# Vanlightly/vsr-tlaplus

Measured on NVIDIA B200. Metric: unique states explored/sec (VSR.tla, shipped VSR.cfg constants), higher is better.
Workload: dtype u32

## Files before the change

### vsr-tlaplus_b200/csrc/vsr_gpu.cuh

```cuda
#ifndef VSR_GPU_CUH
#define VSR_GPU_CUH

#include <cuda_runtime.h>
#include <stdint.h>

#include "vsr_actions.h"

namespace vsr {

struct DevCounters {
    unsigned long long out_count;
    unsigned long long generated;
    unsigned long long ties;
    unsigned long long collisions;
    unsigned long long probes;
    unsigned long long viol_id;
    unsigned long long dead_id;
    unsigned long long tie_count;
    int error;
    int overflow;
    int viol_which;
    int _pad;
    unsigned long long work_next;
    unsigned long long drain_next;
    unsigned int send_count[8];
};

struct TieRec {
    uint64_t fp;
    uint64_t parent;
    uint32_t auxkey, cand, check, _pad;
};

struct RecHdr {
    uint64_t fp;
    uint64_t tm;
};
constexpr int MAX_WORLD = 8;


struct ExpandParams {
    const uint32_t* in;
    unsigned long long n_in;
    unsigned long long in_base;
    const uint32_t* in_hi;
    unsigned long long in_split;
    uint32_t* out;
    uint32_t* out_hi;
    unsigned long long out_split;
    unsigned long long out_cap;
    unsigned long long out_base;
    uint64_t* table;
    unsigned long long table_cap;
    uint64_t* trace;
    unsigned long long trace_cap;
    DevCounters* ctr;
    uint8_t* ties;
    unsigned long long tie_cap;
    const uint64_t* fp_tab;
    RunCfg run;
    int level;
    int check_deadlock;
    int rank, world, owner_shift;
    uint8_t* push[MAX_WORLD];
    unsigned long long push_cap;
    int push_direct;
    const uint8_t* drain[MAX_WORLD];
    unsigned int drain_n[MAX_WORLD];
    unsigned long long drain_total;
};

struct InsertParams {
    const uint8_t* recs;
    unsigned long long n;
    ExpandParams e;
};


__device__ __forceinline__ void cas128(uint64_t* p, uint64_t s0, uint64_t s1, uint64_t& o0, uint64_t& o1) {
    asm volatile(
        "{\n\t.reg .b128 cmp, swp, old;\n\tmov.b128 cmp, {%2, %3};\n\tmov.b128 swp, {%4, %5};\n\t"
        "atom.global.relaxed.gpu.cas.b128 old, [%6], cmp, swp;\n\tmov.b128 {%0, %1}, old;\n\t}"
        : "=l"(o0), "=l"(o1)
        : "l"(0ull), "l"(0ull), "l"(s0), "l"(s1), "l"(p)
        : "memory");
}
__device__ __forceinline__ void ld128_cg(const uint64_t* p, uint64_t& a, uint64_t& b) {
    asm volatile("ld.global.cg.v2.u64 {%0, %1}, [%2];" : "=l"(a), "=l"(b) : "l"(p) : "memory");
}
__device__ __forceinline__ uint64_t mix64(uint64_t x) {
    x ^= x >> 30; x *= 0xbf58476d1ce4e5b9ULL;
    x ^= x >> 27; x *= 0x94d049bb133111ebULL;
    x ^= x >> 31;
    return x;
}
template <class L, bool USE_VIEW, class W> VSR_HD uint32_t check_hash_t(const W& w) {
    constexpr int full = L::VIEW_BITS >> 5, rem = L::VIEW_BITS & 31;
    constexpr int nw = USE_VIEW ? (full + (rem ? 1 : 0)) : L::NW;
    uint32_t h = 0x9747b28cu;
VSR_UNROLL
    for (int i = 0; i < nw; i++) {
        uint32_t k = rdw(w, i);
        if (USE_VIEW && i == full) k &= (1u << rem) - 1u;
        h ^= k;
        h = ((h << 13) | (h >> 19)) * 5u + 0xe6546b64u;
    }
    h ^= h >> 16; h *= 0x85ebca6bu; h ^= h >> 13; h *= 0xc2b2ae35u; h ^= h >> 16;
    return h;
}
template <class L, class W> VSR_HD uint32_t check_hash(const W& w, bool use_view) {
    return use_view ? check_hash_t<L, true>(w) : check_hash_t<L, false>(w);
}

enum { INS_NEW = 0, INS_DUP = 1, INS_TIE = 2, INS_FULL = 3 };

constexpr unsigned long long GID_MASK = (1ull << 44) - 1ull, ROOT_GID = GID_MASK;
__host__ __device__ __forceinline__ uint64_t make_gid(int rank, unsigned long long local_id) { return ((uint64_t)rank << 40) | local_id; }
__host__ __device__ __forceinline__ uint64_t make_trec(uint64_t parent_gid, uint32_t cand) { return (parent_gid << 12) | (cand & 0xFFFu); }

__device__ __forceinline__ uint64_t make_meta(int level, uint32_t auxkey, uint32_t check) {
    return ((uint64_t)(uint32_t)level << 56) | ((uint64_t)(auxkey & 0xFFFFFFu) << 32) | check;
}

#ifndef VSR_BUCKET
#define VSR_BUCKET 2
#endif
struct Probe { uint64_t e[2 * VSR_BUCKET]; };
__device__ __forceinline__ void ld256_cg(const uint64_t* p, uint64_t& a, uint64_t& b, uint64_t& c, uint64_t& d) {
    asm volatile("ld.global.cg.v4.u64 {%0, %1, %2, %3}, [%4];" : "=l"(a), "=l"(b), "=l"(c), "=l"(d) : "l"(p) : "memory");
}
__device__ __forceinline__ unsigned long long table_home(unsigned long long cap, uint64_t fp) {
    return __umul64hi(fp * 0x9E3779B97F4A7C15ULL, cap / VSR_BUCKET) * VSR_BUCKET;
}
__device__ __forceinline__ void probe_load(const uint64_t* table, unsigned long long h, Probe& p) {
#if VSR_BUCKET == 1
    ld128_cg(table + 2 * h, p.e[0], p.e[1]);
#elif VSR_BUCKET == 2
    ld256_cg(table + 2 * h, p.e[0], p.e[1], p.e[2], p.e[3]);
#elif VSR_BUCKET == 4
    ld256_cg(table + 2 * h, p.e[0], p.e[1], p.e[2], p.e[3]);
    ld256_cg(table + 2 * h + 4, p.e[4], p.e[5], p.e[6], p.e[7]);
#else
#error "VSR_BUCKET must be 1, 2 or 4"
#endif
}
__device__ __forceinline__ int table_insert_from(uint64_t* table, unsigned long long cap, unsigned long long h, Probe p, uint64_t fp, uint64_t meta,
                                                 unsigned& probes, unsigned& collisions) {
    for (unsigned tries = 0;; tries++) {
        if (tries > (1u << 16)) return INS_FULL;
        probes++;
VSR_UNROLL
        for (int j = 0; j < VSR_BUCKET; j++) {
            uint64_t e0 = p.e[2 * j], e1 = p.e[2 * j + 1];
            if (e0 == 0) {
                cas128(table + 2 * (h + j), fp, meta, e0, e1);
                if (e0 == 0 && e1 == 0) return INS_NEW;
            }
            for (int again = 0; e1 == 0 && again < 64; again++) ld128_cg(table + 2 * (h + j), e0, e1);
            if (e0 == fp) {
                if ((uint32_t)e1 == (uint32_t)meta) {
                    const bool same_level = (e1 >> 56) == (meta >> 56);
                    const bool same_aux = ((e1 >> 32) & 0xFFFFFF) == ((meta >> 32) & 0xFFFFFF);
                    return (same_level && !same_aux) ? INS_TIE : INS_DUP;
                }
                collisions++;
            }
        }
        h += VSR_BUCKET;
        if (h >= cap) h = 0;
        probe_load(table, h, p);
    }
}
#if defined(VSR_EXP_CASFIRST) && VSR_BUCKET == 2
__device__ __forceinline__ int table_insert_casfirst(uint64_t* table, unsigned long long cap, unsigned long long h, uint64_t fp, uint64_t meta,
                                                     unsigned& probes, unsigned& collisions) {
    Probe p;
    cas128(table + 2 * h, fp, meta, p.e[0], p.e[1]);
    if (p.e[0] == 0 && p.e[1] == 0) { probes++; return INS_NEW; }
    if (p.e[0] == fp && (uint32_t)p.e[1] == (uint32_t)meta) {
        probes++;
        const bool same_level = (p.e[1] >> 56) == (meta >> 56);
        const bool same_aux = ((p.e[1] >> 32) & 0xFFFFFF) == ((meta >> 32) & 0xFFFFFF);
        return (same_level && !same_aux) ? INS_TIE : INS_DUP;
    }
    ld128_cg(table + 2 * (h + 1), p.e[2], p.e[3]);
    return table_insert_from(table, cap, h, p, fp, meta, probes, collisions);
}
#endif
__device__ __forceinline__ int table_insert(uint64_t* table, unsigned long long cap, uint64_t fp, uint64_t meta,
                                            unsigned& probes, unsigned& collisions) {
    const unsigned long long h = table_home(cap, fp);
    Probe p;
    probe_load(table, h, p);
    return table_insert_from(table, cap, h, p, fp, meta, probes, collisions);
}

__device__ __forceinline__ void bulk_store(void* gdst, const void* ssrc, uint32_t bytes) {
    asm volatile("fence.proxy.async.shared::cta;" ::: "memory");
    const uint32_t s = (uint32_t)__cvta_generic_to_shared(ssrc);
    asm volatile("cp.async.bulk.global.shared::cta.bulk_group [%0], [%1], %2;" ::"l"(gdst), "r"(s), "r"(bytes) : "memory");
    asm volatile("cp.async.bulk.commit_group;" ::: "memory");
    asm volatile("cp.async.bulk.wait_group.read 0;" ::: "memory");
}

template <int NW> __device__ __forceinline__ uint32_t* out_state(const ExpandParams& P, unsigned long long i) {
    return i < P.out_split ? P.out + i * NW : P.out_hi + (i - P.out_split) * NW;
}


constexpr int SCAP = 64;
#ifdef VSR_QPS
constexpr int QPS = VSR_QPS;
#else
constexpr int QPS = 10;
#endif

template <class L> struct WarpStage {
    alignas(16) uint32_t stage[SCAP * L::NW + 32];
    unsigned long long tstage[SCAP];
    int sn;
};
template <class L, int WARPS> struct BlockSmemT {
    static constexpr int NS = WARPS * 32;
    static constexpr int NG = 13;
    uint64_t fp_tab[8 * 256];
    uint32_t par[NS * (L::NW + 1)];
    static constexpr int QCAP = QPS * NS;
    uint16_t pool[QCAP];
    int qcount[NG];
    int take;
    unsigned long long round_first;
    WarpStage<L> w[WARPS];
};
template <class L> struct ExpandCfg {
    static constexpr size_t SMEM_ONE = 227 * 1024 - 512, SMEM_TWO = 113 * 1024;
    static constexpr int max_grp() { int m = 0; for (int g = 0; g < Ops<L>::NGRP; g++) m = Ops<L>::grp_size(g) > m ? Ops<L>::grp_size(g) : m; return m; }
    template <int W> static constexpr int pick_one() {
        if constexpr (W < 18) return 0;
        else if constexpr (sizeof(BlockSmemT<L, W>) <= SMEM_ONE) return W;
        else return pick_one<W - 2>();
    }
    static constexpr int W2 = sizeof(BlockSmemT<L, 16>) <= SMEM_TWO ? 16 : (sizeof(BlockSmemT<L, 12>) <= SMEM_TWO ? 12 : 8);
    static constexpr int W1 = max_grp() < 64 ? pick_one<32>() : 0;
#ifdef VSR_FORCE_WARPS
    static constexpr int WARPS = VSR_FORCE_WARPS;
#else
    static constexpr int WARPS = W1 >= 2 * W2 - 4 ? W1 : W2;
#endif
    static constexpr int BLOCKS = WARPS > 16 ? 1 : 2;
    typedef BlockSmemT<L, WARPS> Smem;
};

template <class L, bool MULTI> struct Expander {
    typedef Ops<L> O_;
    typedef typename ExpandCfg<L>::Smem Smem;
    static constexpr int WARPS = ExpandCfg<L>::WARPS, NS = Smem::NS;
    const ExpandParams& P;
    Smem& B;
    WarpStage<L>& S;
    const int lane, warp, tid;
    const uint32_t* mine = nullptr;
    bool have = false;

    __device__ Expander(const ExpandParams& p, Smem& b) : P(p), B(b), S(b.w[threadIdx.x >> 5]), lane(threadIdx.x & 31), warp(threadIdx.x >> 5), tid(threadIdx.x) {}

    static __device__ __noinline__ void flush(const ExpandParams& P, WarpStage<L>& S, int lane, int n) {
        const int sn = S.sn;
        unsigned long long base = 0;
        if (lane == 0) base = atomicAdd(&P.ctr->out_count, (unsigned long long)n);
        base = __shfl_sync(0xffffffffu, base, 0);
        if (lane < n) {
            const unsigned long long t = S.tstage[lane];
            if (t >> 63) {
                atomicMin(&P.ctr->viol_id, P.out_base + base + lane);
                S.tstage[lane] = t & ~(1ull << 63);
            }
        }
        __syncwarp();
        if (base + n > P.out_cap) {
            if (lane == 0) atomicExch(&P.ctr->overflow, 1);
        } else {
            if (lane == 0) {
                if (base + n <= P.out_split) bulk_store(P.out + base * L::NW, S.stage, (uint32_t)(n * L::BYTES));
                else if (base >= P.out_split) bulk_store(P.out_hi + (base - P.out_split) * L::NW, S.stage, (uint32_t)(n * L::BYTES));
                else {
                    const int n1 = (int)(P.out_split - base);
                    bulk_store(P.out + base * L::NW, S.stage, (uint32_t)(n1 * L::BYTES));
                    bulk_store(P.out_hi, S.stage + n1 * L::NW, (uint32_t)((n - n1) * L::BYTES));
                }
            }
            if (P.trace && lane < n && P.out_base + base + lane < P.trace_cap) P.trace[P.out_base + base + lane] = S.tstage[lane];
        }
        __syncwarp();
        const int rest = sn - n;
        for (int i0 = 0; i0 < rest * L::NW; i0 += 32) {
            const int i = i0 + lane;
            uint32_t v = 0;
            if (i < rest * L::NW) v = S.stage[n * L::NW + i];
            __syncwarp();
            if (i < rest * L::NW) S.stage[i] = v;
        }
        unsigned long long t = 0;
        if (lane < rest) t = S.tstage[n + lane];
        __syncwarp();
        if (lane < rest) S.tstage[lane] = t;
        if (lane == 0) S.sn = rest;
        __syncwarp();
    }

    typedef uint32_t* Row;
    static constexpr int gcd32(int a) { int g = 32; while (a % g) g >>= 1; return g; }
    static constexpr int SKEW_P = 32 / gcd32(L::NW);
    static __device__ __forceinline__ Row scratch(WarpStage<L>& S, int lane) { return &S.stage[(32 + lane) * L::NW + lane / SKEW_P]; }

    static __device__ __forceinline__ void push_records(const ExpandParams& P, WarpStage<L>& S, int lane, const RegRow<L::NW>& v, int send_to, uint64_t fp,
                                                        uint64_t tm) {
        const unsigned senders = __ballot_sync(0xffffffffu, send_to >= 0);
        if (!senders) return;
        constexpr int RB = L::BYTES + (int)sizeof(RecHdr), RW = RB / 4;
        constexpr int CAPREC = (32 * L::BYTES) / RB;
        static_assert(CAPREC >= 16, "two passes must cover a batch");
        int off = 0, cnt = 0, rnk = 0;
        unsigned mymask = 0;
        for (int d = 0; d < P.world; d++) {
            const unsigned m = __ballot_sync(0xffffffffu, send_to == d);
            if (send_to > d) off += __popc(m);
            if (send_to == d) { mymask = m; cnt = __popc(m); rnk = __popc(m & ((1u << lane) - 1u)); }
        }
        unsigned base = 0;
        if (send_to >= 0 && rnk == 0) base = atomicAdd(&P.ctr->send_count[send_to], (unsigned)cnt);
        base = __shfl_sync(0xffffffffu, base, mymask ? __ffs(mymask) - 1 : 0);
        const bool fits = send_to >= 0 && (unsigned long long)base + (unsigned)cnt <= P.push_cap;
        if (send_to >= 0 && !fits && rnk == 0) atomicExch(&P.ctr->overflow, 3);
        if (P.push_direct) {
            if (fits) {
                uint4* d = reinterpret_cast<uint4*>(P.push[send_to] + (size_t)(base + (unsigned)rnk) * RB);
                VSR_UNROLL
                for (int q = 0; q < L::NW / 4; q++) d[q] = make_uint4(v.w[4 * q], v.w[4 * q + 1], v.w[4 * q + 2], v.w[4 * q + 3]);
                d[L::NW / 4] = make_uint4((uint32_t)fp, (uint32_t)(fp >> 32), (uint32_t)tm, (uint32_t)(tm >> 32));
            }
            return;
        }
        const int pos = off + rnk, total = __popc(senders);
        uint32_t* sbuf = &S.stage[32 * L::NW];
        for (int lo = 0; lo < total; lo += CAPREC) {
            const int hi = lo + CAPREC < total ? lo + CAPREC : total;
            if (send_to >= 0 && pos >= lo && pos < hi) {
                uint32_t* r = sbuf + (pos - lo) * RW;
                VSR_UNROLL
                for (int j = 0; j < L::NW; j++) r[j] = v.w[j];
                r[L::NW] = (uint32_t)fp; r[L::NW + 1] = (uint32_t)(fp >> 32);
                r[L::NW + 2] = (uint32_t)tm; r[L::NW + 3] = (uint32_t)(tm >> 32);
            }
            __syncwarp();
            if (fits) {
                const int st = off > lo ? off : lo, en = off + cnt < hi ? off + cnt : hi;
                if (pos == st && st < en)
                    bulk_store(P.push[send_to] + (size_t)(base + (unsigned)(st - off)) * RB, sbuf + (st - lo) * RW, (uint32_t)((en - st) * RB));
            }
            __syncwarp();
        }
    }

    static __device__ __forceinline__ unsigned long long commit(const ExpandParams& P, WarpStage<L>& S, int lane, const RegRow<L::NW>& v, bool live, uint64_t fp,
                                                                uint32_t chk, uint32_t auxkey, unsigned long long home, const Probe& first, unsigned long long trec,
                                                                unsigned mult, bool check_inv = true) {
        unsigned gen = 0, probes = 0, coll = 0;
        int sn = S.sn;
        bool isnew = false;
        int bad = 0;
        if (live) {
            const uint64_t meta = make_meta(P.level, auxkey, chk);
            gen = mult;
#if defined(VSR_EXP_CASFIRST) && VSR_BUCKET == 2
            (void)first;
            const int r = table_insert_casfirst(P.table, P.table_cap, home, fp, meta, probes, coll);
#else
            const int r = table_insert_from(P.table, P.table_cap, home, first, fp, meta, probes, coll);
#endif
            isnew = r == INS_NEW;
            if (r == INS_FULL) atomicExch(&P.ctr->overflow, 4);
            if (isnew && check_inv) bad = O_::invariant(P.run, v);
            if (coll) atomicAdd(&P.ctr->collisions, (unsigned long long)coll);
            if (r == INS_TIE) {
                atomicAdd(&P.ctr->ties, 1ull);
                const unsigned long long t = atomicAdd(&P.ctr->tie_count, 1ull);
                if (t < P.tie_cap) {
                    TieRec rec;
                    rec.fp = fp; rec.parent = trec >> 12; rec.auxkey = auxkey; rec.cand = (uint32_t)(trec & 0xFFFu); rec.check = chk; rec._pad = 0;
                    uint8_t* dst = P.ties + t * (sizeof(TieRec) + L::BYTES);
                    *(TieRec*)dst = rec;
                    VSR_UNROLL
                    for (int j = 0; j < L::NW; j++) ((uint32_t*)(dst + sizeof(TieRec)))[j] = v.w[j];
                } else atomicExch(&P.ctr->overflow, 2);
            }
        }
        const unsigned newmask = __ballot_sync(0xffffffffu, isnew);
        __syncwarp();
        if (isnew) {
            const int slot = sn + __popc(newmask & ((1u << lane) - 1u));
            VSR_UNROLL
            for (int j = 0; j < L::NW; j++) S.stage[slot * L::NW + j] = v.w[j];
            if (bad) {
                trec |= 1ull << 63;
                atomicOr(&P.ctr->viol_which, bad);
            }
            S.tstage[slot] = trec;
        }
        sn += __popc(newmask);
        __syncwarp();
        if (lane == 0) S.sn = sn;
        __syncwarp();
        while (sn >= 32) {
            flush(P, S, lane, 32);
            sn -= 32;
        }
        return (unsigned long long)gen | ((unsigned long long)probes << 32);
    }

    static __device__ __noinline__ unsigned long long emit(const ExpandParams& P, Smem& B, WarpStage<L>& S, int lane, const Row n, int mult,
                                                           int cand, int si, bool act, bool check_inv) {
        int send_to = -1;
        uint64_t fp = 0;
        uint32_t chk = 0, auxkey = 0;
        unsigned long long home = 0, trec = 0;
        Probe first = {};
        bool live = false;
        RegRow<L::NW> v;
        if (act && mult > 0) {
            VSR_UNROLL
            for (int j = 0; j < L::NW; j++) v.w[j] = rdw(n, j);
        }
        if (act) {
            if (mult < 0) {
                atomicCAS(&P.ctr->error, 0, mult);
            } else if (mult > 0) {
                fp = fp64_view8<L>(B.fp_tab, v, P.run.use_view != 0);
                if (fp == 0) fp = 1;
                const int owner = MULTI ? owner_of(fp, P.owner_shift) : P.rank;
                trec = make_trec(make_gid(P.rank, P.in_base + B.round_first + si), (uint32_t)cand);
                if (owner == P.rank) {
                    live = true;
                    home = table_home(P.table_cap, fp);
#if !(defined(VSR_EXP_CASFIRST) && VSR_BUCKET == 2)
                    probe_load(P.table, home, first);
#endif
                    chk = check_hash<L>(v, P.run.use_view != 0);
                    auxkey = O_::aux_key(v);
                } else {
                    send_to = owner;
                }
            }
        }
        if (MULTI) {
            __syncwarp();
            push_records(P, S, lane, v, send_to, fp, trec | ((uint64_t)(unsigned)mult << 56));
        }
        return commit(P, S, lane, v, live, fp, chk, auxkey, home, first, trec, (unsigned)mult, check_inv);
    }

    struct DrainPre {
        uint64_t fp, tm;
        unsigned long long home;
        Probe first;
        const uint4* rec;
        bool have;
    };
    unsigned long long dchunk = ~0ull;
    __device__ __forceinline__ unsigned long long drain_chunks() const { return (P.drain_total + 31) / 32; }
    __device__ __forceinline__ unsigned long long drain_claim() {
        unsigned long long c = 0;
        if (lane == 0) c = atomicAdd(&P.ctr->drain_next, 1ull);
        return c;
    }
    __device__ __forceinline__ DrainPre drain_begin(unsigned long long chunk) {
        constexpr int RB = L::BYTES + (int)sizeof(RecHdr);
        DrainPre d;
        unsigned long long i = chunk * 32 + lane;
        d.have = chunk < drain_chunks() && i < P.drain_total;
        d.fp = d.tm = 0;
        d.home = 0;
        d.first = Probe{};
        d.rec = nullptr;
        if (d.have) {
            int s = 0;
            while (s < P.world - 1 && i >= P.drain_n[s]) { i -= P.drain_n[s]; s++; }
            d.rec = reinterpret_cast<const uint4*>(P.drain[s] + i * RB);
            const uint4 h = __ldcs(d.rec + L::NW / 4);
            d.fp = ((uint64_t)h.y << 32) | h.x;
            d.tm = ((uint64_t)h.w << 32) | h.z;
            d.home = table_home(P.table_cap, d.fp);
#if !(defined(VSR_EXP_CASFIRST) && VSR_BUCKET == 2)
            probe_load(P.table, d.home, d.first);
#endif
        }
        return d;
    }
    __device__ __forceinline__ void drain_end(const DrainPre& d) {
        RegRow<L::NW> v;
        uint32_t chk = 0, auxkey = 0;
        if (d.have) {
            VSR_UNROLL
            for (int q = 0; q < L::NW / 4; q++) {
                const uint4 x = __ldcs(d.rec + q);
                v.w[4 * q] = x.x; v.w[4 * q + 1] = x.y; v.w[4 * q + 2] = x.z; v.w[4 * q + 3] = x.w;
            }
            chk = check_hash<L>(v, P.run.use_view != 0);
            auxkey = O_::aux_key(v);
        }
        tally(commit(P, S, lane, v, d.have, d.fp, chk, auxkey, d.home, d.first, d.tm & ((1ull << 56) - 1ull), (unsigned)((d.tm >> 56) & 0xFu)));
    }
    __device__ void drain() {
        const unsigned long long nchunks = drain_chunks();
        if (dchunk == ~0ull) dchunk = __shfl_sync(0xffffffffu, drain_claim(), 0);
        while (dchunk < nchunks) {
            const unsigned long long nx = drain_claim();
            const DrainPre d = drain_begin(dchunk);
            drain_end(d);
            dchunk = __shfl_sync(0xffffffffu, nx, 0);
        }
    }

    static constexpr int NG = O_::NGRP;
    static __host__ __device__ constexpr int moff(int g) { int o = 0; for (int h = 0; h < g; h++) o += O_::grp_words(h); return o; }
    static constexpr int MW = moff(NG);
    static constexpr int PW = (NG + 1) / 2;
    static __host__ __device__ constexpr int max_grp() { int m = 0; for (int g = 0; g < NG; g++) m = O_::grp_size(g) > m ? O_::grp_size(g) : m; return m; }
    static constexpr int TBITS = NS <= 512 ? 9 : 10;
    static_assert(NS <= (1 << TBITS) && max_grp() < (1 << (16 - TBITS)), "pool item does not fit 16 bits");
    static_assert(max_grp() * NS < 65536, "16-bit packed counters");

    template <int G> __device__ __forceinline__ void guards(const RegRow<L::NW>& st, uint32_t* m, uint32_t* pc) {
        O_::template enabled_group<G>(P.run, st, m + moff(G));
        uint32_t c = 0;
        VSR_UNROLL
        for (int k = 0; k < O_::grp_words(G); k++) c += (uint32_t)__popc(m[moff(G) + k]);
        pc[G >> 1] += c << (16 * (G & 1));
        if constexpr (G + 1 < NG) guards<G + 1>(st, m, pc);
    }
    template <int G, bool FAST> __device__ __forceinline__ void push(uint32_t* m, const uint32_t* ex, const uint32_t* wb, int st) {
        int pos = st + (int)((wb[G >> 1] >> (16 * (G & 1))) & 0xFFFFu) + (int)((ex[G >> 1] >> (16 * (G & 1))) & 0xFFFFu);
        VSR_UNROLL
        for (int k = 0; k < O_::grp_words(G); k++) {
            uint32_t mm = m[moff(G) + k], left = 0;
            while (mm) {
                const int bit = __ffs(mm) - 1;
                mm &= mm - 1;
                if (FAST || pos < Smem::QCAP) B.pool[pos] = (uint16_t)(tid | ((k * 32 + bit) << TBITS));
                else left |= 1u << bit;
                pos++;
            }
            if (!FAST) m[moff(G) + k] = left;
        }
        if constexpr (G + 1 < NG) {
            const int nst = FAST ? st + B.qcount[G] : (st + B.qcount[G] < Smem::QCAP ? st + B.qcount[G] : Smem::QCAP);
            push<G + 1, FAST>(m, ex, wb, nst);
        }
    }
    template <int G> __device__ __forceinline__ void leftovers(uint32_t* m) {
        VSR_UNROLL
        for (int k = 0; k < O_::grp_words(G); k++) {
            while (__any_sync(0xffffffffu, m[moff(G) + k] != 0)) {
                const bool inl = m[moff(G) + k] != 0;
                int cand = 0;
                if (inl) {
                    const int bit = __ffs(m[moff(G) + k]) - 1;
                    m[moff(G) + k] &= m[moff(G) + k] - 1;
                    cand = O_::grp_begin(G) + k * 32 + bit;
                }
                tally(apply<G>(P, B, S, lane, mine, cand, tid, inl));
            }
        }
        if constexpr (G + 1 < NG) leftovers<G + 1>(m);
    }
    __device__ __forceinline__ void scan_all() {
        uint32_t m[MW], pc[PW];
        VSR_UNROLL
        for (int i = 0; i < MW; i++) m[i] = 0;
        VSR_UNROLL
        for (int i = 0; i < PW; i++) pc[i] = 0;
        if (have) {
            RegRow<L::NW> st;
            VSR_UNROLL
            for (int i = 0; i < L::NW; i++) st.w[i] = mine[i];
            guards<0>(st, m, pc);
        }
        uint32_t ex[PW], wb[PW];
        VSR_UNROLL
        for (int i = 0; i < PW; i++) ex[i] = pc[i];
        VSR_UNROLL
        for (int o = 1; o < 32; o <<= 1) {
            VSR_UNROLL
            for (int i = 0; i < PW; i++) {
                const uint32_t t = __shfl_up_sync(0xffffffffu, ex[i], o);
                if (lane >= o) ex[i] += t;
            }
        }
        uint32_t mytot = 0, anyc = 0;
        VSR_UNROLL
        for (int g = 0; g < NG; g++) {
            const uint32_t t = (__shfl_sync(0xffffffffu, ex[g >> 1], 31) >> (16 * (g & 1))) & 0xFFFFu;
            if (lane == g) mytot = t;
        }
        VSR_UNROLL
        for (int i = 0; i < PW; i++) { anyc |= pc[i]; ex[i] -= pc[i]; }
        uint32_t mybase = 0;
        if (lane < NG && mytot) mybase = (uint32_t)atomicAdd(&B.qcount[lane], (int)mytot);
        VSR_UNROLL
        for (int i = 0; i < PW; i++) wb[i] = 0;
        VSR_UNROLL
        for (int g = 0; g < NG; g++) wb[g >> 1] |= (__shfl_sync(0xffffffffu, mybase, g) & 0xFFFFu) << (16 * (g & 1));
        if (P.check_deadlock && have && !anyc) atomicMin(&P.ctr->dead_id, P.in_base + B.round_first + tid);
        __syncthreads();
#ifndef VSR_EXP_NO_PUSHFAST
        int all = 0;
        VSR_UNROLL
        for (int g = 0; g < NG; g++) all += B.qcount[g];
        if (all <= Smem::QCAP) {
            push<0, true>(m, ex, wb, 0);
            return;
        }
#endif
        push<0, false>(m, ex, wb, 0);
        uint32_t rest = 0;
        VSR_UNROLL
        for (int i = 0; i < MW; i++) rest |= m[i];
        if (__any_sync(0xffffffffu, rest != 0)) leftovers<0>(m);
    }
    template <int G> static __device__ __noinline__ unsigned long long apply(const ExpandParams& P, Smem& B, WarpStage<L>& S, int lane,
                                                                             const uint32_t* parent, int cand, int si, bool act) {
        const Row n = scratch(S, lane);
        int mult = 0;
        if (act) mult = O_::template step_grp<true, G>(P.run, parent, cand, n);
#ifdef VSR_EXP_INVSKIP
        return emit(P, B, S, lane, n, mult, cand, si, act, O_::may_falsify(G));
#else
        return emit(P, B, S, lane, n, mult, cand, si, act, true);
#endif
    }
    template <int G> static __device__ __forceinline__ unsigned long long batch(const ExpandParams& P, Smem& B, WarpStage<L>& S, int lane, int b,
                                                                                int k) {
        const bool act = lane < k;
        int cand = 0, si = 0;
        if (act) {
            const unsigned item = B.pool[b + lane];
            si = item & ((1 << TBITS) - 1);
            cand = O_::grp_begin(G) + (int)(item >> TBITS);
        }
        return apply<G>(P, B, S, lane, &B.par[si * (L::NW + 1)], cand, si, act);
    }
    unsigned long long acc_gen = 0, acc_probes = 0;
    __device__ __forceinline__ void tally(unsigned long long r) {
        acc_gen += (unsigned)r;
        acc_probes += r >> 32;
    }

    __device__ void run_round(unsigned long long first, int count) {
        const uint32_t* src = P.in + first * L::NW;
        if (first + count <= P.in_split) {
            for (int i = tid; i < count * L::NW; i += NS) B.par[(i / L::NW) * (L::NW + 1) + (i % L::NW)] = __ldg(src + i);
        } else {
            for (int i = tid; i < count * L::NW; i += NS) {
                const unsigned long long st = first + i / L::NW;
                const uint32_t* row = st < P.in_split ? P.in + st * L::NW : P.in_hi + (st - P.in_split) * L::NW;
                B.par[(i / L::NW) * (L::NW + 1) + (i % L::NW)] = __ldg(row + i % L::NW);
            }
        }
        if (tid < Smem::NG) B.qcount[tid] = 0;
        if (tid == 0) { B.round_first = first; B.take = 0; }
        __syncthreads();
        have = tid < count;
        mine = &B.par[(have ? tid : 0) * (L::NW + 1)];
        scan_all();
        __syncthreads();
        const int q = lane < Smem::NG ? B.qcount[lane] : 0;
        int inc = q;
        VSR_UNROLL
        for (int o = 1; o < 32; o <<= 1) {
            const int t = __shfl_up_sync(0xffffffffu, inc, o);
            if (lane >= o) inc += t;
        }
        const int seg_st = inc - q < Smem::QCAP ? inc - q : Smem::QCAP, seg_en = inc < Smem::QCAP ? inc : Smem::QCAP;
        const int nb = (seg_en - seg_st + 31) >> 5;
        int binc = nb;
        VSR_UNROLL
        for (int o = 1; o < 32; o <<= 1) {
            const int t = __shfl_up_sync(0xffffffffu, binc, o);
            if (lane >= o) binc += t;
        }
        const int total = __shfl_sync(0xffffffffu, binc, 31);
        for (;;) {
            int t = 0;
            if (lane == 0) t = atomicAdd(&B.take, 1);
            t = __shfl_sync(0xffffffffu, t, 0);
            if (t >= total) break;
            const int g = __popc(__ballot_sync(0xffffffffu, lane < Smem::NG && binc <= t));
            const int st = __shfl_sync(0xffffffffu, seg_st, g), en = __shfl_sync(0xffffffffu, seg_en, g);
            const int b = st + (t - __shfl_sync(0xffffffffu, binc - nb, g)) * 32;
            const int k = en - b < 32 ? en - b : 32;
            unsigned long long r;
            switch (g) {
            case 0: r = batch<0>(P, B, S, lane, b, k); break;   case 1: r = batch<1>(P, B, S, lane, b, k); break;
            case 2: r = batch<2>(P, B, S, lane, b, k); break;   case 3: r = batch<3>(P, B, S, lane, b, k); break;
            case 4: r = batch<4>(P, B, S, lane, b, k); break;   case 5: r = batch<5>(P, B, S, lane, b, k); break;
            case 6: r = batch<6>(P, B, S, lane, b, k); break;   case 7: r = batch<7>(P, B, S, lane, b, k); break;
            case 8: r = batch<8>(P, B, S, lane, b, k); break;   case 9: r = batch<9>(P, B, S, lane, b, k); break;
            case 10: r = batch<10>(P, B, S, lane, b, k); break; case 11: r = batch<11>(P, B, S, lane, b, k); break;
            default: r = batch<12>(P, B, S, lane, b, k); break;
            }
            tally(r);
        }
    }

    __device__ void finish() {
        while (S.sn > 0) flush(P, S, lane, S.sn < 32 ? S.sn : 32);
        for (int o = 16; o; o >>= 1) {
            acc_gen += __shfl_xor_sync(0xffffffffu, acc_gen, o);
            acc_probes += __shfl_xor_sync(0xffffffffu, acc_probes, o);
        }
        if (lane == 0) {
            atomicAdd(&P.ctr->generated, acc_gen);
            atomicAdd(&P.ctr->probes, acc_probes);
        }
    }
};

template <class L, bool MULTI> __global__ void __launch_bounds__(ExpandCfg<L>::WARPS * 32, ExpandCfg<L>::BLOCKS) expand_kernel(const __grid_constant__ ExpandParams P) {
    extern __shared__ __align__(128) unsigned char smem_raw[];
    typedef typename ExpandCfg<L>::Smem Smem;
    Smem& B = *reinterpret_cast<Smem*>(smem_raw);
    for (int i = threadIdx.x; i < 8 * 256; i += blockDim.x) B.fp_tab[i] = P.fp_tab[i];
    __shared__ unsigned long long next_round;
    Expander<L, MULTI> X(P, B);
    if ((threadIdx.x & 31) == 0) {
        WarpStage<L>& S = B.w[threadIdx.x >> 5];
        S.sn = 0;
    }
    const unsigned long long nrounds = (P.n_in + Smem::NS - 1) / Smem::NS;
    if (threadIdx.x == 0) next_round = atomicAdd(&P.ctr->work_next, 1ull);
    for (;;) {
        __syncthreads();
        const unsigned long long c = next_round;
        __syncthreads();
        if (c >= nrounds) break;
        if (threadIdx.x == 0) {
            next_round = atomicAdd(&P.ctr->work_next, 1ull);
            const unsigned long long nx = next_round;
            if (nx < nrounds && (nx + 1) * Smem::NS <= P.in_split) {
                const unsigned long long nfirst = nx * Smem::NS;
                const unsigned long long ncount = (P.n_in - nfirst) < (unsigned long long)Smem::NS ? (P.n_in - nfirst) : Smem::NS;
                asm volatile("cp.async.bulk.prefetch.L2.global [%0], %1;" ::"l"(P.in + nfirst * L::NW), "r"((uint32_t)(ncount * L::BYTES)) : "memory");
            }
        }
        const unsigned long long first = c * Smem::NS;
        const int count = (int)((P.n_in - first) < (unsigned long long)Smem::NS ? (P.n_in - first) : Smem::NS);
        X.run_round(first, count);
    }
    if (MULTI && P.drain_total) X.drain();
    X.finish();
}


template <class L> __global__ void __launch_bounds__(256) insert_kernel(const InsertParams Q) {
    const ExpandParams& P = Q.e;
    const unsigned long long i = (unsigned long long)blockIdx.x * blockDim.x + threadIdx.x;
    const int lane = threadIdx.x & 31;
    const bool have = i < Q.n;
    bool isnew = false;
    const uint8_t* rec = Q.recs + (have ? i : 0) * (L::BYTES + sizeof(RecHdr));
    const uint32_t* n = (const uint32_t*)rec;
    const RecHdr* h = (const RecHdr*)(rec + L::BYTES);
    unsigned probes = 0, coll = 0, nties = 0;
    unsigned long long gen = 0;
    uint64_t parent = 0;
    uint32_t cand = 0;
    if (have) {
        const uint64_t meta = make_meta(P.level, Ops<L>::aux_key(n), check_hash<L>(n, P.run.use_view != 0));
        const int r = table_insert(P.table, P.table_cap, h->fp, meta, probes, coll);
        isnew = r == INS_NEW;
        if (r == INS_FULL) atomicExch(&P.ctr->overflow, 4);
        gen = (h->tm >> 56) & 0xFu;
        parent = (h->tm >> 12) & ((1ull << 44) - 1ull);
        cand = (uint32_t)(h->tm & 0xFFFu);
        if (r == INS_TIE) {
            nties = 1;
            const unsigned long long t = atomicAdd(&P.ctr->tie_count, 1ull);
            if (t < P.tie_cap) {
                TieRec tr;
                tr.fp = h->fp; tr.parent = parent; tr.auxkey = (uint32_t)((meta >> 32) & 0xFFFFFF); tr.cand = cand;
                tr.check = (uint32_t)meta; tr._pad = 0;
                uint8_t* dst = P.ties + t * (sizeof(TieRec) + L::BYTES);
                *(TieRec*)dst = tr;
                for (int j = 0; j < L::NW; j++) ((uint32_t*)(dst + sizeof(TieRec)))[j] = n[j];
            } else atomicExch(&P.ctr->overflow, 2);
        }
    }
    for (int o = 16; o; o >>= 1) {
        gen += __shfl_xor_sync(0xffffffffu, gen, o);
        probes += __shfl_xor_sync(0xffffffffu, probes, o);
        coll += __shfl_xor_sync(0xffffffffu, coll, o);
        nties += __shfl_xor_sync(0xffffffffu, nties, o);
    }
    if (lane == 0) {
        if (gen) atomicAdd(&P.ctr->generated, gen);
        if (probes) atomicAdd(&P.ctr->probes, (unsigned long long)probes);
        if (coll) atomicAdd(&P.ctr->collisions, (unsigned long long)coll);
        if (nties) atomicAdd(&P.ctr->ties, (unsigned long long)nties);
    }
    const unsigned newmask = __ballot_sync(0xffffffffu, isnew);
    if (newmask) {
        unsigned long long base = 0;
        const int leader = __ffs(newmask) - 1;
        if (lane == leader) base = atomicAdd(&P.ctr->out_count, (unsigned long long)__popc(newmask));
        base = __shfl_sync(0xffffffffu, base, leader);
        if (isnew) {
            const unsigned long long pos = base + __popc(newmask & ((1u << lane) - 1u));
            if (pos < P.out_cap) {
                uint32_t* dst = out_state<L::NW>(P, pos);
                for (int j = 0; j < L::NW; j++) dst[j] = n[j];
                if (P.trace && P.out_base + pos < P.trace_cap) P.trace[P.out_base + pos] = make_trec(parent, cand);
                const int bad = Ops<L>::invariant(P.run, n);
                if (bad) {
                    atomicMin(&P.ctr->viol_id, P.out_base + pos);
                    atomicOr(&P.ctr->viol_which, bad);
                }
            } else atomicExch(&P.ctr->overflow, 1);
        }
    }
}

template <class L> __global__ void patch_ties_kernel(const ExpandParams P, const uint8_t* ties, unsigned long long ntie, unsigned long long n_out) {
    const unsigned long long i = (unsigned long long)blockIdx.x * blockDim.x + threadIdx.x;
    if (i >= n_out) return;
    uint32_t w[L::NW];
    uint32_t* st = out_state<L::NW>(P, i);
    for (int j = 0; j < L::NW; j++) w[j] = st[j];
    uint64_t fp = fp64_view8<L>(P.fp_tab, w, P.run.use_view != 0);
    if (fp == 0) fp = 1;
    const uint32_t chk = check_hash<L>(w, P.run.use_view != 0);
    const size_t stride = sizeof(TieRec) + L::BYTES;
    unsigned long long lo = 0, hi = ntie;
    while (lo < hi) {
        const unsigned long long mid = (lo + hi) / 2;
        if (((const TieRec*)(ties + mid * stride))->fp < fp) lo = mid + 1; else hi = mid;
    }
    for (; lo < ntie; lo++) {
        const TieRec* t = (const TieRec*)(ties + lo * stride);
        if (t->fp != fp) break;
        if (t->check != chk) continue;
        if (t->auxkey < Ops<L>::aux_key(w)) {
            const uint32_t* tw = (const uint32_t*)((const uint8_t*)t + sizeof(TieRec));
            for (int j = 0; j < L::NW; j++) { w[j] = tw[j]; st[j] = tw[j]; }
            if (P.trace && P.out_base + i < P.trace_cap) P.trace[P.out_base + i] = make_trec(t->parent, t->cand);
        }
    }
    const int bad = Ops<L>::invariant(P.run, w);
    if (bad) {
        atomicMin(&P.ctr->viol_id, P.out_base + i);
        atomicOr(&P.ctr->viol_which, bad);
    }
}

static __global__ void lookup_kernel(const uint64_t* table, unsigned long long cap, uint64_t fp, uint32_t check, unsigned long long* meta_out) {
    unsigned long long h = table_home(cap, fp);
    for (unsigned long long i = 0; i < cap; i++) {
        const uint64_t e0 = table[2 * h], e1 = table[2 * h + 1];
        if (e0 == 0) { *meta_out = 0; return; }
        if (e0 == fp && (uint32_t)e1 == check) { *meta_out = e1; return; }
        if (++h >= cap) h = 0;
    }
    *meta_out = 0;
}

struct SimParams {
    unsigned long long num_walks, seed;
    int depth;
    RunCfg run;
    unsigned long long* first_bad;
    unsigned long long* steps;
    unsigned long long* dead_ends;
    unsigned long long* probe_out;
    unsigned long long probe_walks;
    const uint64_t* fp_tab;
};
template <class L> __global__ void simulate_kernel(const SimParams Q) {
    unsigned long long steps = 0, dead = 0;
    for (unsigned long long wk = (unsigned long long)blockIdx.x * blockDim.x + threadIdx.x; wk < Q.num_walks; wk += (unsigned long long)gridDim.x * blockDim.x) {
        uint64_t rng = Q.seed ^ (wk * 0xD1B54A32D192ED03ULL);
        uint32_t a[L::NW], b[L::NW];
        Ops<L>::init((uint32_t*)a);
        unsigned long long mysteps = 0;
        for (int d = 2; d <= Q.depth; d++) {
            const int cand = Ops<L>::random_enabled(Q.run, (const uint32_t*)a, rng);
            if (cand < 0) { dead++; break; }
            if (Ops<L>::template step<true>(Q.run, (const uint32_t*)a, cand, (uint32_t*)b) <= 0) break;
            for (int j = 0; j < L::NW; j++) a[j] = b[j];
            steps++;
            mysteps++;
            if (Ops<L>::invariant(Q.run, (const uint32_t*)a)) {
                atomicMin(Q.first_bad, (wk << 16) | (unsigned long long)d);
                break;
            }
        }
        if (wk < Q.probe_walks) {
            Q.probe_out[2 * wk] = fp64_view<L>(Q.fp_tab, (const uint32_t*)a, false);
            Q.probe_out[2 * wk + 1] = mysteps;
        }
    }
    for (int o = 16; o; o >>= 1) {
        steps += __shfl_xor_sync(0xffffffffu, steps, o);
        dead += __shfl_xor_sync(0xffffffffu, dead, o);
    }
    if ((threadIdx.x & 31) == 0) {
        atomicAdd(Q.steps, steps);
        atomicAdd(Q.dead_ends, dead);
    }
}

static __global__ void probe_bench_kernel(uint64_t* table, unsigned long long cap, unsigned long long n, unsigned long long distinct,
                                   unsigned long long seed, unsigned long long* new_count, unsigned long long* probe_count) {
    unsigned long long mine_new = 0;
    unsigned probes = 0, coll = 0;
    for (unsigned long long i = (unsigned long long)blockIdx.x * blockDim.x + threadIdx.x; i < n; i += (unsigned long long)gridDim.x * blockDim.x) {
        unsigned long long z = seed + (i % distinct) * 0x9E3779B97F4A7C15ULL;
        z = (z ^ (z >> 30)) * 0xBF58476D1CE4E5B9ULL;
        z = (z ^ (z >> 27)) * 0x94D049BB133111EBULL;
        z ^= z >> 31;
        if (z == 0) z = 1;
        mine_new += table_insert(table, cap, z, make_meta(1, 0, (uint32_t)(z >> 32) | 1u), probes, coll) == INS_NEW;
    }
    for (int o = 16; o; o >>= 1) {
        mine_new += __shfl_xor_sync(0xffffffffu, mine_new, o);
        probes += __shfl_xor_sync(0xffffffffu, probes, o);
    }
    if ((threadIdx.x & 31) == 0) {
        atomicAdd(new_count, mine_new);
        atomicAdd(probe_count, (unsigned long long)probes);
    }
}

}
#endif
```

Baseline: 3.864 billion.

## Software-pipeline successor emission and write new states directly to global output

Each warp now double-buffers successor rows in shared memory and defers the hash-table insert of one batch until the next batch's successors have been generated, so the table probe load overlaps with the next step computation. The per-warp staging buffer with bulk-copy flushes is removed. New states get their output slot from an atomic right away and are stored straight to global memory with vector stores, and the invariant check moves after the insert. This adds pending-state bookkeeping and an extra settle call at the end of each round, and it trades coalesced bulk copies for scattered per-lane stores.

```diff
diff --git a/vsr-tlaplus_b200/csrc/vsr_gpu.cuh b/vsr-tlaplus_b200/csrc/vsr_gpu.cuh
--- a/vsr-tlaplus_b200/csrc/vsr_gpu.cuh
+++ b/vsr-tlaplus_b200/csrc/vsr_gpu.cuh
@@ -117,6 +117,7 @@
 constexpr unsigned long long GID_MASK = (1ull << 44) - 1ull, ROOT_GID = GID_MASK;
 __host__ __device__ __forceinline__ uint64_t make_gid(int rank, unsigned long long local_id) { return ((uint64_t)rank << 40) | local_id; }
 __host__ __device__ __forceinline__ uint64_t make_trec(uint64_t parent_gid, uint32_t cand) { return (parent_gid << 12) | (cand & 0xFFFu); }
+constexpr uint64_t TM_NOINV = 1ull << 63;
 
 __device__ __forceinline__ uint64_t make_meta(int level, uint32_t auxkey, uint32_t check) {
     return ((uint64_t)(uint32_t)level << 56) | ((uint64_t)(auxkey & 0xFFFFFFu) << 32) | check;
@@ -207,18 +208,32 @@
     return i < P.out_split ? P.out + i * NW : P.out_hi + (i - P.out_split) * NW;
 }
 
-
-constexpr int SCAP = 64;
+template <int NW> __device__ __forceinline__ void store_state(uint32_t* dst, const RegRow<NW>& v) {
+    if constexpr (NW % 4 == 0) {
+        VSR_UNROLL
+        for (int q = 0; q < NW / 4; q++) reinterpret_cast<uint4*>(dst)[q] = make_uint4(v.w[4 * q], v.w[4 * q + 1], v.w[4 * q + 2], v.w[4 * q + 3]);
+    } else if constexpr (NW % 2 == 0) {
+        VSR_UNROLL
+        for (int q = 0; q < NW / 2; q++) reinterpret_cast<uint2*>(dst)[q] = make_uint2(v.w[2 * q], v.w[2 * q + 1]);
+    } else {
+        VSR_UNROLL
+        for (int j = 0; j < NW; j++) dst[j] = v.w[j];
+    }
+}
+
+
 #ifdef VSR_QPS
 constexpr int QPS = VSR_QPS;
 #else
 constexpr int QPS = 10;
 #endif
 
+constexpr int gcd32(int a) { int g = 32; while (a % g) g >>= 1; return g; }
 template <class L> struct WarpStage {
-    alignas(16) uint32_t stage[SCAP * L::NW + 32];
-    unsigned long long tstage[SCAP];
-    int sn;
+    static constexpr int SKEW_P = 32 / gcd32(L::NW);
+    static constexpr int SET_W = (32 * L::NW + 31 / SKEW_P + 3) & ~3;
+    alignas(16) uint32_t set[2][SET_W];
+    RecHdr pend[32];
 };
 template <class L, int WARPS> struct BlockSmemT {
     static constexpr int NS = WARPS * 32;
@@ -264,59 +279,21 @@
 
     __device__ Expander(const ExpandParams& p, Smem& b) : P(p), B(b), S(b.w[threadIdx.x >> 5]), lane(threadIdx.x & 31), warp(threadIdx.x >> 5), tid(threadIdx.x) {}
 
-    static __device__ __noinline__ void flush(const ExpandParams& P, WarpStage<L>& S, int lane, int n) {
-        const int sn = S.sn;
-        unsigned long long base = 0;
-        if (lane == 0) base = atomicAdd(&P.ctr->out_count, (unsigned long long)n);
-        base = __shfl_sync(0xffffffffu, base, 0);
-        if (lane < n) {
-            const unsigned long long t = S.tstage[lane];
-            if (t >> 63) {
-                atomicMin(&P.ctr->viol_id, P.out_base + base + lane);
-                S.tstage[lane] = t & ~(1ull << 63);
-            }
-        }
-        __syncwarp();
-        if (base + n > P.out_cap) {
-            if (lane == 0) atomicExch(&P.ctr->overflow, 1);
-        } else {
-            if (lane == 0) {
-                if (base + n <= P.out_split) bulk_store(P.out + base * L::NW, S.stage, (uint32_t)(n * L::BYTES));
-                else if (base >= P.out_split) bulk_store(P.out_hi + (base - P.out_split) * L::NW, S.stage, (uint32_t)(n * L::BYTES));
-                else {
-                    const int n1 = (int)(P.out_split - base);
-                    bulk_store(P.out + base * L::NW, S.stage, (uint32_t)(n1 * L::BYTES));
-                    bulk_store(P.out_hi, S.stage + n1 * L::NW, (uint32_t)((n - n1) * L::BYTES));
-                }
-            }
-            if (P.trace && lane < n && P.out_base + base + lane < P.trace_cap) P.trace[P.out_base + base + lane] = S.tstage[lane];
-        }
-        __syncwarp();
-        const int rest = sn - n;
-        for (int i0 = 0; i0 < rest * L::NW; i0 += 32) {
-            const int i = i0 + lane;
-            uint32_t v = 0;
-            if (i < rest * L::NW) v = S.stage[n * L::NW + i];
-            __syncwarp();
-            if (i < rest * L::NW) S.stage[i] = v;
-        }
-        unsigned long long t = 0;
-        if (lane < rest) t = S.tstage[n + lane];
-        __syncwarp();
-        if (lane < rest) S.tstage[lane] = t;
-        if (lane == 0) S.sn = rest;
-        __syncwarp();
-    }
-
     typedef uint32_t* Row;
-    static constexpr int gcd32(int a) { int g = 32; while (a % g) g >>= 1; return g; }
-    static constexpr int SKEW_P = 32 / gcd32(L::NW);
-    static __device__ __forceinline__ Row scratch(WarpStage<L>& S, int lane) { return &S.stage[(32 + lane) * L::NW + lane / SKEW_P]; }
-
-    static __device__ __forceinline__ void push_records(const ExpandParams& P, WarpStage<L>& S, int lane, const RegRow<L::NW>& v, int send_to, uint64_t fp,
-                                                        uint64_t tm) {
+    static __device__ __forceinline__ Row scratch(WarpStage<L>& S, int lane, int set) {
+        return &S.set[set][lane * L::NW + lane / WarpStage<L>::SKEW_P];
+    }
+
+    static __device__ __forceinline__ void push_records(const ExpandParams& P, WarpStage<L>& S, int lane, int set) {
+        const uint64_t fp = S.pend[lane].fp, tm = S.pend[lane].tm & ~TM_NOINV;
+        int send_to = -1;
+        if (tm) {
+            const int owner = owner_of(fp, P.owner_shift);
+            if (owner != P.rank) send_to = owner;
+        }
         const unsigned senders = __ballot_sync(0xffffffffu, send_to >= 0);
         if (!senders) return;
+        const Row n = scratch(S, lane, set);
         constexpr int RB = L::BYTES + (int)sizeof(RecHdr), RW = RB / 4;
         constexpr int CAPREC = (32 * L::BYTES) / RB;
         static_assert(CAPREC >= 16, "two passes must cover a batch");
@@ -336,19 +313,19 @@
             if (fits) {
                 uint4* d = reinterpret_cast<uint4*>(P.push[send_to] + (size_t)(base + (unsigned)rnk) * RB);
                 VSR_UNROLL
-                for (int q = 0; q < L::NW / 4; q++) d[q] = make_uint4(v.w[4 * q], v.w[4 * q + 1], v.w[4 * q + 2], v.w[4 * q + 3]);
+                for (int q = 0; q < L::NW / 4; q++) d[q] = make_uint4(n[4 * q], n[4 * q + 1], n[4 * q + 2], n[4 * q + 3]);
                 d[L::NW / 4] = make_uint4((uint32_t)fp, (uint32_t)(fp >> 32), (uint32_t)tm, (uint32_t)(tm >> 32));
             }
             return;
         }
         const int pos = off + rnk, total = __popc(senders);
-        uint32_t* sbuf = &S.stage[32 * L::NW];
+        uint32_t* sbuf = S.set[set ^ 1];
         for (int lo = 0; lo < total; lo += CAPREC) {
             const int hi = lo + CAPREC < total ? lo + CAPREC : total;
             if (send_to >= 0 && pos >= lo && pos < hi) {
                 uint32_t* r = sbuf + (pos - lo) * RW;
                 VSR_UNROLL
-                for (int j = 0; j < L::NW; j++) r[j] = v.w[j];
+                for (int j = 0; j < L::NW; j++) r[j] = n[j];
                 r[L::NW] = (uint32_t)fp; r[L::NW + 1] = (uint32_t)(fp >> 32);
                 r[L::NW + 2] = (uint32_t)tm; r[L::NW + 3] = (uint32_t)(tm >> 32);
             }
@@ -362,13 +339,11 @@
         }
     }
 
-    static __device__ __forceinline__ unsigned long long commit(const ExpandParams& P, WarpStage<L>& S, int lane, const RegRow<L::NW>& v, bool live, uint64_t fp,
+    static __device__ __forceinline__ unsigned long long commit(const ExpandParams& P, int lane, const RegRow<L::NW>& v, bool live, uint64_t fp,
                                                                 uint32_t chk, uint32_t auxkey, unsigned long long home, const Probe& first, unsigned long long trec,
                                                                 unsigned mult, bool check_inv = true) {
         unsigned gen = 0, probes = 0, coll = 0;
-        int sn = S.sn;
         bool isnew = false;
-        int bad = 0;
         if (live) {
             const uint64_t meta = make_meta(P.level, auxkey, chk);
             gen = mult;
@@ -380,7 +355,6 @@
 #endif
             isnew = r == INS_NEW;
             if (r == INS_FULL) atomicExch(&P.ctr->overflow, 4);
-            if (isnew && check_inv) bad = O_::invariant(P.run, v);
             if (coll) atomicAdd(&P.ctr->collisions, (unsigned long long)coll);
             if (r == INS_TIE) {
                 atomicAdd(&P.ctr->ties, 1ull);
@@ -396,67 +370,72 @@
             }
         }
         const unsigned newmask = __ballot_sync(0xffffffffu, isnew);
-        __syncwarp();
-        if (isnew) {
-            const int slot = sn + __popc(newmask & ((1u << lane) - 1u));
-            VSR_UNROLL
-            for (int j = 0; j < L::NW; j++) S.stage[slot * L::NW + j] = v.w[j];
-            if (bad) {
-                trec |= 1ull << 63;
-                atomicOr(&P.ctr->viol_which, bad);
-            }
-            S.tstage[slot] = trec;
-        }
-        sn += __popc(newmask);
-        __syncwarp();
-        if (lane == 0) S.sn = sn;
-        __syncwarp();
-        while (sn >= 32) {
-            flush(P, S, lane, 32);
-            sn -= 32;
+        if (newmask) {
+            unsigned long long base = 0;
+            if (lane == 0) base = atomicAdd(&P.ctr->out_count, (unsigned long long)__popc(newmask));
+            int bad = 0;
+            if (isnew && check_inv) bad = O_::invariant(P.run, v);
+            base = __shfl_sync(0xffffffffu, base, 0);
+            if (isnew) {
+                const unsigned long long pos = base + __popc(newmask & ((1u << lane) - 1u));
+                if (pos < P.out_cap) {
+                    store_state<L::NW>(out_state<L::NW>(P, pos), v);
+                    if (P.trace && P.out_base + pos < P.trace_cap) P.trace[P.out_base + pos] = trec;
+                } else atomicExch(&P.ctr->overflow, 1);
+                if (bad) {
+                    atomicMin(&P.ctr->viol_id, P.out_base + pos);
+                    atomicOr(&P.ctr->viol_which, bad);
+                }
+            }
         }
         return (unsigned long long)gen | ((unsigned long long)probes << 32);
     }
 
-    static __device__ __noinline__ unsigned long long emit(const ExpandParams& P, Smem& B, WarpStage<L>& S, int lane, const Row n, int mult,
+    static __device__ __noinline__ unsigned long long emit(const ExpandParams& P, Smem& B, WarpStage<L>& S, int lane, int set, bool pending, int mult,
                                                            int cand, int si, bool act, bool check_inv) {
-        int send_to = -1;
-        uint64_t fp = 0;
-        uint32_t chk = 0, auxkey = 0;
-        unsigned long long home = 0, trec = 0;
-        Probe first = {};
-        bool live = false;
-        RegRow<L::NW> v;
-        if (act && mult > 0) {
-            VSR_UNROLL
-            for (int j = 0; j < L::NW; j++) v.w[j] = rdw(n, j);
-        }
+        uint64_t fp = 0, tm = 0;
         if (act) {
             if (mult < 0) {
                 atomicCAS(&P.ctr->error, 0, mult);
             } else if (mult > 0) {
+                const Row n = scratch(S, lane, set);
+                RegRow<L::NW> v;
+                VSR_UNROLL
+                for (int j = 0; j < L::NW; j++) v.w[j] = n[j];
                 fp = fp64_view8<L>(B.fp_tab, v, P.run.use_view != 0);
                 if (fp == 0) fp = 1;
-                const int owner = MULTI ? owner_of(fp, P.owner_shift) : P.rank;
-                trec = make_trec(make_gid(P.rank, P.in_base + B.round_first + si), (uint32_t)cand);
-                if (owner == P.rank) {
-                    live = true;
-                    home = table_home(P.table_cap, fp);
+                tm = make_trec(make_gid(P.rank, P.in_base + B.round_first + si), (uint32_t)cand) | ((uint64_t)(unsigned)mult << 56) | (check_inv ? 0ull : TM_NOINV);
+            }
+        }
+        const uint64_t pfp = S.pend[lane].fp, ptm = S.pend[lane].tm;
+        S.pend[lane].fp = fp;
+        S.pend[lane].tm = tm;
+        unsigned long long r = 0;
+        if (pending) {
+            bool live = ptm != 0;
+            if (MULTI && live) live = owner_of(pfp, P.owner_shift) == P.rank;
+            unsigned long long home = 0;
+            Probe first = {};
+            RegRow<L::NW> v;
+            uint32_t chk = 0, auxkey = 0;
+            if (live) {
+                home = table_home(P.table_cap, pfp);
 #if !(defined(VSR_EXP_CASFIRST) && VSR_BUCKET == 2)
-                    probe_load(P.table, home, first);
-#endif
-                    chk = check_hash<L>(v, P.run.use_view != 0);
-                    auxkey = O_::aux_key(v);
-                } else {
-                    send_to = owner;
-                }
-            }
+                probe_load(P.table, home, first);
+#endif
+                const Row n = scratch(S, lane, set ^ 1);
+                VSR_UNROLL
+                for (int j = 0; j < L::NW; j++) v.w[j] = n[j];
+                chk = check_hash<L>(v, P.run.use_view != 0);
+                auxkey = O_::aux_key(v);
+            }
+            r = commit(P, lane, v, live, pfp, chk, auxkey, home, first, ptm & ((1ull << 56) - 1ull), (unsigned)((ptm >> 56) & 0xFu), !(ptm & TM_NOINV));
         }
         if (MULTI) {
             __syncwarp();
-            push_records(P, S, lane, v, send_to, fp, trec | ((uint64_t)(unsigned)mult << 56));
-        }
-        return commit(P, S, lane, v, live, fp, chk, auxkey, home, first, trec, (unsigned)mult, check_inv);
+            push_records(P, S, lane, set);
+        }
+        return r;
     }
 
     struct DrainPre {
@@ -508,7 +487,7 @@
             chk = check_hash<L>(v, P.run.use_view != 0);
             auxkey = O_::aux_key(v);
         }
-        tally(commit(P, S, lane, v, d.have, d.fp, chk, auxkey, d.home, d.first, d.tm & ((1ull << 56) - 1ull), (unsigned)((d.tm >> 56) & 0xFu)));
+        tally(commit(P, lane, v, d.have, d.fp, chk, auxkey, d.home, d.first, d.tm & ((1ull << 56) - 1ull), (unsigned)((d.tm >> 56) & 0xFu)));
     }
     __device__ void drain() {
         const unsigned long long nchunks = drain_chunks();
@@ -568,7 +547,8 @@
                     m[moff(G) + k] &= m[moff(G) + k] - 1;
                     cand = O_::grp_begin(G) + k * 32 + bit;
                 }
-                tally(apply<G>(P, B, S, lane, mine, cand, tid, inl));
+                tally(apply<G>(P, B, S, lane, cur, pend, mine, cand, tid, inl));
+                applied();
             }
         }
         if constexpr (G + 1 < NG) leftovers<G + 1>(m);
@@ -627,19 +607,19 @@
         for (int i = 0; i < MW; i++) rest |= m[i];
         if (__any_sync(0xffffffffu, rest != 0)) leftovers<0>(m);
     }
-    template <int G> static __device__ __noinline__ unsigned long long apply(const ExpandParams& P, Smem& B, WarpStage<L>& S, int lane,
-                                                                             const uint32_t* parent, int cand, int si, bool act) {
-        const Row n = scratch(S, lane);
+    template <int G> static __device__ __noinline__ unsigned long long apply(const ExpandParams& P, Smem& B, WarpStage<L>& S, int lane, int set,
+                                                                             bool pending, const uint32_t* parent, int cand, int si, bool act) {
+        const Row n = scratch(S, lane, set);
         int mult = 0;
         if (act) mult = O_::template step_grp<true, G>(P.run, parent, cand, n);
 #ifdef VSR_EXP_INVSKIP
-        return emit(P, B, S, lane, n, mult, cand, si, act, O_::may_falsify(G));
+        return emit(P, B, S, lane, set, pending, mult, cand, si, act, O_::may_falsify(G));
 #else
-        return emit(P, B, S, lane, n, mult, cand, si, act, true);
-#endif
-    }
-    template <int G> static __device__ __forceinline__ unsigned long long batch(const ExpandParams& P, Smem& B, WarpStage<L>& S, int lane, int b,
-                                                                                int k) {
+        return emit(P, B, S, lane, set, pending, mult, cand, si, act, true);
+#endif
+    }
+    template <int G> static __device__ __forceinline__ unsigned long long batch(const ExpandParams& P, Smem& B, WarpStage<L>& S, int lane, int set,
+                                                                                bool pending, int b, int k) {
         const bool act = lane < k;
         int cand = 0, si = 0;
         if (act) {
@@ -647,12 +627,24 @@
             si = item & ((1 << TBITS) - 1);
             cand = O_::grp_begin(G) + (int)(item >> TBITS);
         }
-        return apply<G>(P, B, S, lane, &B.par[si * (L::NW + 1)], cand, si, act);
+        return apply<G>(P, B, S, lane, set, pending, &B.par[si * (L::NW + 1)], cand, si, act);
     }
     unsigned long long acc_gen = 0, acc_probes = 0;
     __device__ __forceinline__ void tally(unsigned long long r) {
         acc_gen += (unsigned)r;
         acc_probes += r >> 32;
+    }
+    int cur = 0;
+    bool pend = false;
+    __device__ __forceinline__ void applied() {
+        cur ^= 1;
+        pend = true;
+    }
+    __device__ __forceinline__ void settle() {
+        if (pend) {
+            tally(emit(P, B, S, lane, cur, true, 0, 0, 0, false, true));
+            pend = false;
+        }
     }
 
     __device__ void run_round(unsigned long long first, int count) {
@@ -700,20 +692,21 @@
             const int k = en - b < 32 ? en - b : 32;
             unsigned long long r;
             switch (g) {
-            case 0: r = batch<0>(P, B, S, lane, b, k); break;   case 1: r = batch<1>(P, B, S, lane, b, k); break;
-            case 2: r = batch<2>(P, B, S, lane, b, k); break;   case 3: r = batch<3>(P, B, S, lane, b, k); break;
-            case 4: r = batch<4>(P, B, S, lane, b, k); break;   case 5: r = batch<5>(P, B, S, lane, b, k); break;
-            case 6: r = batch<6>(P, B, S, lane, b, k); break;   case 7: r = batch<7>(P, B, S, lane, b, k); break;
-            case 8: r = batch<8>(P, B, S, lane, b, k); break;   case 9: r = batch<9>(P, B, S, lane, b, k); break;
-            case 10: r = batch<10>(P, B, S, lane, b, k); break; case 11: r = batch<11>(P, B, S, lane, b, k); break;
-            default: r = batch<12>(P, B, S, lane, b, k); break;
+            case 0: r = batch<0>(P, B, S, lane, cur, pend, b, k); break;   case 1: r = batch<1>(P, B, S, lane, cur, pend, b, k); break;
+            case 2: r = batch<2>(P, B, S, lane, cur, pend, b, k); break;   case 3: r = batch<3>(P, B, S, lane, cur, pend, b, k); break;
+            case 4: r = batch<4>(P, B, S, lane, cur, pend, b, k); break;   case 5: r = batch<5>(P, B, S, lane, cur, pend, b, k); break;
+            case 6: r = batch<6>(P, B, S, lane, cur, pend, b, k); break;   case 7: r = batch<7>(P, B, S, lane, cur, pend, b, k); break;
+            case 8: r = batch<8>(P, B, S, lane, cur, pend, b, k); break;   case 9: r = batch<9>(P, B, S, lane, cur, pend, b, k); break;
+            case 10: r = batch<10>(P, B, S, lane, cur, pend, b, k); break; case 11: r = batch<11>(P, B, S, lane, cur, pend, b, k); break;
+            default: r = batch<12>(P, B, S, lane, cur, pend, b, k); break;
             }
             tally(r);
-        }
+            applied();
+        }
+        settle();
     }
 
     __device__ void finish() {
-        while (S.sn > 0) flush(P, S, lane, S.sn < 32 ? S.sn : 32);
         for (int o = 16; o; o >>= 1) {
             acc_gen += __shfl_xor_sync(0xffffffffu, acc_gen, o);
             acc_probes += __shfl_xor_sync(0xffffffffu, acc_probes, o);
@@ -732,10 +725,6 @@
     for (int i = threadIdx.x; i < 8 * 256; i += blockDim.x) B.fp_tab[i] = P.fp_tab[i];
     __shared__ unsigned long long next_round;
     Expander<L, MULTI> X(P, B);
-    if ((threadIdx.x & 31) == 0) {
-        WarpStage<L>& S = B.w[threadIdx.x >> 5];
-        S.sn = 0;
-    }
     const unsigned long long nrounds = (P.n_in + Smem::NS - 1) / Smem::NS;
     if (threadIdx.x == 0) next_round = atomicAdd(&P.ctr->work_next, 1ull);
     for (;;) {
```

Result: faster. 3.923 billion, median of 6 (+1.5%).
